# AKASH2907/pi-consistency-activity-detection

Measured on AMD Instinct MI355X. Metric: train clips/sec (bs=8, 16×224×224, I3D+caps+bv cons) at 1/2/4/8 GPU, higher is better.
Workload: dtype f32 (fp32 operands and fp32 accumulation everywhere; 33 of the 79 conv / input-gradient launches and the 3x3x3 / 1x1x1 weight gradients multiply on the bf16 matrix cores: every fp32 operand as the exact sum of 3 bf16 terms, 6 products on v_mfma_f32_32x32x16_bf16, hi / lo fp32 accumulators -- error v

## Files before the change

include/picons.h:

```cpp
#ifndef PICONS_H
#define PICONS_H
#include <stdint.h>
#ifdef __cplusplus
extern "C" {
#endif

typedef void* pc_stream;

#define PC_OK            0
#define PC_E_ARG        -1
#define PC_E_LAUNCH     -2
#define PC_E_NODEVICE   -3

#define PC_ACT_NONE 0
#define PC_ACT_RELU 1
#define PC_ACT_SIGMOID 2

#define PC_F_ACCUM   1
#define PC_F_BIAS    2
#define PC_F_CSCALE  4
#define PC_F_BNPART  8
#define PC_F_NFAST   16
#define PC_F_TOUT    32
#define PC_F_CI3     64
// ... 127 lines not shown
int64_t pc_act_bwd_ws_floats(int64_t rows, int C);
int pc_act_bwd(const float* dy, int lddy, const float* y, int ldy, int act, int C, int64_t rows,
               float* dz, int lddz, float* dbias, int accum, float* ws, pc_stream s);
int pc_ncdhw_to_ndhwc(const void* src, int src_is_f64, int N, int C, int64_t thw, int W, int Cpad,
                      int flipw, float* dst, pc_stream s);
int pc_ndhwc_to_ncdhw(const float* src, int ld, int N, int C, int64_t thw, float* dst, pc_stream s);
int pc_transpose_batched(const float* src, int batch, int R, int Cc, int64_t src_batch_stride,
                         int src_ld, float* dst, int64_t dst_batch_stride, int dst_ld, int accum,
                         pc_stream s);
typedef struct pc_transpose_job {
    uint64_t src, dst;
    int64_t  src_batch_stride, dst_batch_stride;
    int32_t  batch, R, C, src_ld, dst_ld, accum;
    int32_t  nslices, reserved;
    int64_t  slice_stride;
} pc_transpose_job;
int pc_transpose_multi(const pc_transpose_job* jobs, int njobs, pc_stream s);
int pc_col2im(const float* cols, int N, int Ho, int Wo, int KH, int KW, int C, float* dx, int lddx,
              int accum, pc_stream s);
int pc_seg_frame_counts(const float* logits, const float* gt, int64_t nframes, int64_t pix, int32_t* counts, pc_stream s);
int pc_map_accumulate(const int32_t* counts, int64_t nframes, int label, int ncls, int32_t* frame_hits, int32_t* video_hits,
                      int32_t* n_frames, int32_t* n_vids, pc_stream s);
int     pc_val_record_words(int B);
int64_t pc_val_metrics_ws_floats(int B, int64_t pix);
int     pc_val_metrics(const float* output, const float* loc_msk, const float* predicted_action, const int32_t* action, int B, int64_t pix,
                       int C, int32_t* record, float* ws, pc_stream s);
int pc_clip_from_u8(const uint8_t* video, int F, int H, int W, const int32_t* span8, int h0, int w0, int S,
                    const int32_t* rects, int R, float* data, float* aug, float* mask, pc_stream s);
int pc_clip_from_u8_masks(const uint8_t* video, int F, int H, int W, const int32_t* span8, int h0, int w0, int S,
                          const uint8_t* maskframes, const int32_t* valid8, float* data, float* aug, float* mask, float* mask_cls,
                          pc_stream s);
int pc_clip_from_u8_ndhwc4(const uint8_t* video, int F, int H, int W, const int32_t* span8, int h0, int w0, int S,
                           const int32_t* rects, int R, float* data, float* aug, float* mask, pc_stream s);
int pc_truth_frame_flags(const uint8_t* truth, int F, int H, int W, int h0, int w0, int S, int32_t* flags, pc_stream s);
int pc_eval_clips_from_u8(const uint8_t* video, const uint8_t* truth, int F, int H, int W, int h0, int w0, int S,
                          const int32_t* starts, int n, int f_skip, float* data, float* gt, pc_stream s);
int pc_video_vote(const float* pred, int n, int C, int label, int32_t* n_correct, pc_stream s);
int     pc_clips_from_u8(const uint8_t* video, int F, int H, int W, int h0, int w0, int S, const int32_t* starts, int n, int f_skip,
                         float* data, pc_stream s);
int64_t pc_detect_frames_ws_bytes(int n, int S);
int     pc_detect_frames(const float* logits, int F, int H, int W, int h0, int w0, int S, const int32_t* starts, int n, int f_skip,
                         int row0, uint8_t* mask, int32_t* rec, void* ws, pc_stream s);
int     pc_video_class(const float* scores, int n, int C, float* out, pc_stream s);
int     pc_clips_from_u8_views(const uint8_t* video, int F, int H, int W, int S, const int32_t* views, int V, int view_stride,
                               const int32_t* starts, int n, int f_skip, float* data, pc_stream s);
int64_t pc_detect_frames_views_ws_bytes(int n, int H, int W);
int     pc_detect_frames_views(const float* logits, int F, int H, int W, int S, const int32_t* views, int V, int view_stride,
                               const int32_t* starts, int n, int f_skip, int row0, uint8_t* mask, int32_t* rec, void* ws, pc_stream s);
#define PC_INST_HDR      4
#define PC_INST_WORDS    6
#define PC_INST_MAX_RUNS 2048
#define PC_INST_MAX_ROWS 2048
int     pc_frame_instances(const uint8_t* mask, int F, int H, int W, int f0, int nf, int conn, int min_area, int K, int32_t* inst,
                           uint8_t* imap, pc_stream s);
#define PC_PROB_ONE    65535
#define PC_SCORE_WORDS 3
int     pc_frame_probs(const float* logits, int F, int H, int W, int S, const int32_t* views, int V, int view_stride, const int32_t* starts,
                       int n, int f_skip, uint16_t* prob, pc_stream s);
int     pc_instance_scores(const uint8_t* imap, const uint16_t* prob, int F, int H, int W, int f0, int nf, int K, int32_t* out, pc_stream s);
#define PC_LINK_MAX_LAGS 4
int     pc_instance_overlaps(const uint8_t* imap, int F, int H, int W, int f0, int nf, int K, int L, int32_t* out, pc_stream s);
#define PC_RUN_WORDS 2
int64_t pc_mask_run_ws_bytes(int nf, int H);
int     pc_mask_run_index(const uint8_t* map, int F, int H, int W, int f0, int nf, int32_t* index, void* ws, pc_stream s);
int     pc_mask_runs(const uint8_t* map, int F, int H, int W, int f0, int nf, const int32_t* index, int64_t cap, uint32_t* runs, pc_stream s);
#define PC_CROSS_MAX_SLOTS 32
// ... 135 lines not shown
```

pi-consistency-activity-detection_amd/capi.py:

```python
import ctypes as C
import os

import numpy as np

_HERE = os.path.dirname(os.path.abspath(__file__))
DIAG = os.environ.get("PICONS_DIAG_LIB", "0") not in ("", "0")
DIAG_SWITCHES = ("PICONS_CONV_ABLATE", "PICONS_WGRAD_ABLATE", "PICONS_WINO_VARIANT")
LIB_PATH = os.path.join(_HERE, "libpicons_diag.so" if DIAG else "libpicons.so")
if os.environ.get("PICONS_LIB_NAME"):
    LIB_PATH = os.path.join(_HERE, os.path.basename(os.environ["PICONS_LIB_NAME"]))
_lib = None

i32, i64, f32, vp = C.c_int32, C.c_int64, C.c_float, C.c_void_p


class ConvDesc(C.Structure):
    _fields_ = [(n, i32) for n in ("N", "Ti", "Hi", "Wi", "Ci", "ldi", "Tq", "Hq", "Wq", "To", "Ho", "Wo", "Co", "ldo")] + \
               [(n, i32 * 3) for n in ("ostr", "ooff", "istr", "ntap", "ioff0", "istep", "wk0", "wkstep")] + \
               [(n, i32) for n in ("KT", "KH", "KW", "ldw", "act", "flags", "wgstride", "bgstride", "act_c0", "groups")]


class WgradDesc(C.Structure):
    _fields_ = [(n, i32) for n in ("N", "Tq", "Hq", "Wq", "Cd", "ldd", "Ts", "Hs", "Ws", "Cs", "lds")] + \
               [(n, i32 * 3) for n in ("istr", "ntap", "ioff0", "istep", "wk0")] + [(n, i32) for n in ("KT", "KH", "KW", "splitk", "nbatch", "dbstride", "sbstride", "gbstride", "Td", "Hd", "Wd")] + [("doff", i32 * 3), ("flags", i32), ("ws_slices", i32)]
# ... 74 lines not shown
    "pc_wino_weights": (i32, [vp, i64, i64, i64, i32, i32, i32, i32, vp, vp]),
    "pc_wino_weights_multi": (i32, [vp, i32, vp]),
    "pc_wino_conv": (i32, [C.POINTER(WinoDesc), vp, vp, vp, vp, vp, vp]),
    "pc_wino4_u_floats": (i64, [i32, i32, i32]),
    "pc_wino4_weights": (i32, [vp, i64, i64, i64, i32, i32, i32, i32, vp, vp]),
    "pc_wino_bnpart_rows": (i32, [C.POINTER(WinoDesc)]),
    "pc_wino_work": (i32, [C.POINTER(WinoDesc), C.POINTER(C.c_double)]),
    "pc_bn_finalize": (i32, [vp, i32, i32, i32, i64, vp, vp, f32, f32, vp, vp, vp, vp]),
    "pc_bn_finalize_ws": (i32, [vp, i32, i32, i32, i64, vp, vp, f32, f32, vp, vp, vp, vp, vp]),
    "pc_bn_finalize_ws_floats": (i64, [i32, i32, i32]),
    "pc_bn_finalize_apply_ok": (i32, [i32, i32]),
    "pc_bn_finalize_apply": (i32, [vp, i32, i32, i32, i64, vp, vp, f32, f32, vp, vp, vp, vp, i32, i64, vp, i32, i32, vp]),
    "pc_bn_apply": (i32, [vp, i32, vp, i32, i64, i32, vp, i32, i32, vp]),
    "pc_bn_eval_stat": (i32, [vp, vp, vp, vp, f32, i32, vp, vp]),
    "pc_bn_bwd_ws_floats": (i64, [i64, i32, i32]),
    "pc_bn_bwd": (i32, [vp, i32, vp, i32, vp, i32, i64, i32, i32, vp, i32, vp, vp, i32, vp, vp]),
    "pc_maxpool_fwd": (i32, [C.POINTER(PoolDesc), vp, vp, vp, vp]),
    "pc_maxpool_bwd": (i32, [C.POINTER(PoolDesc), vp, vp, vp, i32, vp]),
    "pc_channel_scale": (i32, [vp, i32, vp, i32, i64, i32, vp, i32, i32, vp]),
    "pc_act_bwd_ws_floats": (i64, [i64, i32]),
    "pc_act_bwd": (i32, [vp, i32, vp, i32, i32, i32, i64, vp, i32, vp, i32, vp, vp]),
    "pc_ncdhw_to_ndhwc": (i32, [vp, i32, i32, i32, i64, i32, i32, i32, vp, vp]),
    "pc_ndhwc_to_ncdhw": (i32, [vp, i32, i32, i32, i64, vp, vp]),
    "pc_transpose_batched": (i32, [vp, i32, i32, i32, i64, i32, vp, i64, i32, i32, vp]),
    "pc_col2im": (i32, [vp, i32, i32, i32, i32, i32, i32, vp, i32, i32, vp]),
    "pc_seg_frame_counts": (i32, [vp, vp, i64, i64, vp, vp]),
    "pc_map_accumulate": (i32, [vp, i64, i32, i32, vp, vp, vp, vp, vp]),
    "pc_val_record_words": (i32, [i32]),
    "pc_val_metrics_ws_floats": (i64, [i32, i64]),
    "pc_val_metrics": (i32, [vp, vp, vp, vp, i32, i64, i32, vp, vp, vp]),
    "pc_clip_from_u8": (i32, [vp, i32, i32, i32, C.POINTER(C.c_int32), i32, i32, i32, vp, i32, vp, vp, vp, vp]),
    "pc_clip_from_u8_ndhwc4": (i32, [vp, i32, i32, i32, C.POINTER(C.c_int32), i32, i32, i32, vp, i32, vp, vp, vp, vp]),
    "pc_clip_from_u8_masks": (i32, [vp, i32, i32, i32, C.POINTER(C.c_int32), i32, i32, i32, vp, C.POINTER(C.c_int32), vp, vp, vp, vp, vp]),
    "pc_truth_frame_flags": (i32, [vp, i32, i32, i32, i32, i32, i32, vp, vp]),
    "pc_eval_clips_from_u8": (i32, [vp, vp, i32, i32, i32, i32, i32, i32, C.POINTER(C.c_int32), i32, i32, vp, vp, vp]),
    "pc_video_vote": (i32, [vp, i32, i32, i32, vp, vp]),
    "pc_clips_from_u8": (i32, [vp, i32, i32, i32, i32, i32, i32, C.POINTER(C.c_int32), i32, i32, vp, vp]),
    "pc_detect_frames_ws_bytes": (i64, [i32, i32]),
    "pc_detect_frames": (i32, [vp, i32, i32, i32, i32, i32, i32, C.POINTER(C.c_int32), i32, i32, i32, vp, vp, vp, vp]),
    "pc_video_class": (i32, [vp, i32, i32, vp, vp]),
    "pc_clips_from_u8_views": (i32, [vp, i32, i32, i32, i32, C.POINTER(C.c_int32), i32, i32, C.POINTER(C.c_int32), i32, i32, vp, vp]),
    "pc_detect_frames_views_ws_bytes": (i64, [i32, i32, i32]),
    "pc_detect_frames_views": (i32, [vp, i32, i32, i32, i32, C.POINTER(C.c_int32), i32, i32, C.POINTER(C.c_int32), i32, i32, i32, vp, vp, vp, vp]),
    "pc_frame_instances": (i32, [vp, i32, i32, i32, i32, i32, i32, i32, i32, vp, vp, vp]),
    "pc_frame_probs": (i32, [vp, i32, i32, i32, i32, C.POINTER(C.c_int32), i32, i32, C.POINTER(C.c_int32), i32, i32, vp, vp]),
    "pc_instance_scores": (i32, [vp, vp, i32, i32, i32, i32, i32, i32, vp, vp]),
    "pc_instance_overlaps": (i32, [vp, i32, i32, i32, i32, i32, i32, i32, vp, vp]),
    "pc_mask_run_ws_bytes": (i64, [i32, i32]),
    "pc_mask_run_index": (i32, [vp, i32, i32, i32, i32, i32, vp, vp, vp]),
    "pc_mask_runs": (i32, [vp, i32, i32, i32, i32, i32, vp, i64, vp, vp]),
    "pc_map_crosstab_ws_bytes": (i64, [i32, i32, i32, i32, i32]),
    "pc_map_crosstab": (i32, [vp, vp, i32, i32, i32, i32, i32, i32, i32, vp, vp, vp]),
    "pc_resize_tables": (i64, [i32, i32, i32, i32, i32, vp, i64]),
    "pc_resize_u8": (i32, [vp, i32, i32, i32, i32, i32, i32, vp, i32, vp, vp]),
    "pc_fill": (i32, [vp, i64, f32, vp]),
    "pc_axpy": (i32, [vp, vp, i64, f32, vp]),
    "pc_em_ws_floats": (i64, [i32, i32, i32]),
    "pc_em_state_floats": (i64, [i32]),
    "pc_em_routing_fwd": (i32, [vp, vp, vp, vp, i32, i32, i32, vp, vp, vp]),
    "pc_em_routing_bwd": (i32, [vp, vp, vp, vp, vp, i32, i32, i32, vp, vp, vp, vp, vp, vp, vp]),
    "pc_class_mask_fwd": (i32, [vp, i32, i32, i32, vp, vp, i32, vp, vp, vp, vp]),
    "pc_class_mask_bwd": (i32, [vp, vp, vp, i32, i32, i32, vp, vp]),
    "pc_tapsum_fwd": (i32, [vp, i32, i32, i32, i32, vp, vp, vp]),
    "pc_tapsum_bwd": (i32, [vp, i32, i32, i32, i32, vp, vp]),
    "pc_loss_ws_floats": (i64, [C.POINTER(LossDesc)]),
    "pc_consistency_loss": (i32, [C.POINTER(LossDesc), vp, vp, vp, vp, vp, vp, vp, vp, vp, vp, vp]),
# ... 76 lines not shown
```

pi-consistency-activity-detection_amd/csrc/inputpipe.hip:

```cpp
#include "common.h"
#include <algorithm>
#include <cfloat>
#include <cmath>
#include <cstring>
#include <vector>

namespace {

struct ClipK {
    const uint8_t* video; int F, H, W;
    int span[8]; int h0, w0, S;
    const int32_t* rects; int R;
    const uint8_t* maskf; int valid[8]; float* mask_cls;
    float* data; float* aug; float* mask;
    int nhwc4;
};

__global__ __launch_bounds__(256) void clip_from_u8_kernel(const ClipK p) {
    const int S = p.S;
    const int64_t total = (int64_t)8 * S * S;
    for (int64_t idx = (int64_t)blockIdx.x * 256 + threadIdx.x; idx < total; idx += (int64_t)gridDim.x * 256) {
        const int w = (int)(idx % S), h = (int)((idx / S) % S), t = (int)(idx / ((int64_t)S * S));
        const int f = p.span[t], y = h + p.h0, x = w + p.w0;
        const uint8_t* px = p.video + (((size_t)f * p.H + y) * p.W + x) * 3;
// ... 33 lines not shown
                               const int32_t* rects, int R, float* data, float* aug, float* mask, pc_stream s) {
    return clip_launch(video, F, H, W, span8, h0, w0, S, rects, R, nullptr, nullptr, data, aug, mask, nullptr, s);
}

extern "C" int pc_clip_from_u8_masks(const uint8_t* video, int F, int H, int W, const int32_t* span8, int h0, int w0, int S,
                                     const uint8_t* maskframes, const int32_t* valid8, float* data, float* aug, float* mask, float* mask_cls,
                                     pc_stream s) {
    PC_CHECK_ARG(maskframes && valid8 && mask_cls, "pc_clip_from_u8_masks: null pointer");
    return clip_launch(video, F, H, W, span8, h0, w0, S, nullptr, 0, maskframes, valid8, data, aug, mask, mask_cls, s);
}

extern "C" int pc_clip_from_u8_ndhwc4(const uint8_t* video, int F, int H, int W, const int32_t* span8, int h0, int w0, int S,
                                      const int32_t* rects, int R, float* data, float* aug, float* mask, pc_stream s) {
    PC_CHECK_ARG(((uintptr_t)data % 16 == 0) && ((uintptr_t)aug % 16 == 0), "pc_clip_from_u8_ndhwc4: data / aug must be 16-byte aligned");
    return clip_launch(video, F, H, W, span8, h0, w0, S, rects, R, nullptr, nullptr, data, aug, mask, nullptr, s, 1);
}

static int clip_launch(const uint8_t* video, int F, int H, int W, const int32_t* span8, int h0, int w0, int S, const int32_t* rects, int R,
                       const uint8_t* maskf, const int32_t* valid8, float* data, float* aug, float* mask, float* mask_cls, pc_stream s, int nhwc4) {
    PC_CHECK_ARG(video && span8 && data && aug && mask && (rects || R == 0), "pc_clip_from_u8: null pointer");
    PC_CHECK_ARG(F >= 1 && S >= 1 && h0 >= 0 && w0 >= 0 && h0 + S <= H && w0 + S <= W && R >= 0, "pc_clip_from_u8: crop %d+%d x %d+%d outside %d x %d", h0, S, w0, S, H, W);
    ClipK k;
    k.video = video; k.F = F; k.H = H; k.W = W; k.h0 = h0; k.w0 = w0; k.S = S; k.rects = rects; k.R = R; k.data = data; k.aug = aug; k.mask = mask;
    k.maskf = maskf; k.mask_cls = mask_cls; k.nhwc4 = nhwc4;
    for (int t = 0; t < 8; ++t) k.valid[t] = valid8 ? valid8[t] : 0;
    for (int t = 0; t < 8; ++t) {
        PC_CHECK_ARG(span8[t] >= 0 && span8[t] < F, "pc_clip_from_u8: frame %d outside [0, %d)", span8[t], F);
        k.span[t] = span8[t];
    }
    const int64_t total = (int64_t)8 * S * S;
    int grid = (int)((total + 255) / 256); if (grid > 4096) grid = 4096;
    hipLaunchKernelGGL(clip_from_u8_kernel, dim3(grid), dim3(256), 0, (hipStream_t)s, k);
    PC_CHECK_LAUNCH("clip_from_u8");
    return PC_OK;
}

namespace {

enum { RK_NEAREST = 0, RK_LINEAR = 1, RK_AREA = 2, RK_AREA_FAST = 3, RK_COPY = 4 };
constexpr int RHDR = 8;

inline int cv_floor(double v) { int i = (int)v; return i - (i > v); }
inline int cv_ceil(double v) { int i = (int)v; return i + (i < v); }
inline int32_t fbits(float f) { int32_t b; memcpy(&b, &f, 4); return b; }
inline short sat_short(float v) { long r = lrintf(v); return (short)(r < -32768 ? -32768 : (r > 32767 ? 32767 : r)); }

void area_tab(int ssize, int dsize, double scale, std::vector<int32_t>& start, std::vector<int32_t>& si, std::vector<int32_t>& alpha) {
    for (int dx = 0; dx < dsize; ++dx) {
        start.push_back((int32_t)si.size());
        const double fsx1 = dx * scale, fsx2 = fsx1 + scale;
        const double cell = std::min(scale, ssize - fsx1);
        int sx1 = cv_ceil(fsx1), sx2 = cv_floor(fsx2);
        sx2 = std::min(sx2, ssize - 1);
        sx1 = std::min(sx1, sx2);
        if (sx1 - fsx1 > 1e-3) { si.push_back(sx1 - 1); alpha.push_back(fbits((float)((sx1 - fsx1) / cell))); }
        for (int sx = sx1; sx < sx2; ++sx) { si.push_back(sx); alpha.push_back(fbits(float(1.0 / cell))); }
        if (fsx2 - sx2 > 1e-3) { si.push_back(sx2); alpha.push_back(fbits((float)(std::min(std::min(fsx2 - sx2, 1.), cell) / cell))); }
    }
    start.push_back((int32_t)si.size());
}

struct ResizeK {
    const uint8_t* src; uint8_t* dst; const int32_t* tab;
    int n, H, W, C, Ho, Wo, binarize;
};

// ... 157 lines not shown
```

pi-consistency-activity-detection_amd/inputpipe.py:

```python
import numpy as np
import torch

from . import ops

DEPTH = 8
CROP = 224


class _PinnedRing:

    def __init__(self, depth=24):
        self.depth, self.buf, self.ev, self.nxt = depth, {}, {}, {}

    def _slot(self, shape, dtype):
        kind = (tuple(shape), str(dtype))
        i = self.nxt.get(kind, 0)
        self.nxt[kind] = (i + 1) % self.depth
        key = kind + (i,)
        if key not in self.buf:
            self.buf[key] = torch.empty(tuple(shape), dtype=torch.from_numpy(np.empty(0, dtype)).dtype).pin_memory()
            self.ev[key] = None
        if self.ev[key] is not None:
            self.ev[key].synchronize()
        return key, self.buf[key]

    def _send(self, key, b, device):
        d = b.to(device, non_blocking=True)
        ev = torch.cuda.Event()
        ev.record(torch.cuda.current_stream(d.device))
        self.ev[key] = ev
        return d

    def upload(self, frames, span, device):
        key, b = self._slot((len(span),) + tuple(frames.shape[1:]), frames.dtype)
        bn = b.numpy()
        for t, f in enumerate(span):
            bn[t] = frames[int(f)]
        return self._send(key, b, device)

    def upload_array(self, arr, device):
        key, b = self._slot(arr.shape, arr.dtype)
        b.numpy()[...] = arr
        return self._send(key, b, device)


_ring = _PinnedRing()


def pinned_upload(arr, device):
    return _ring.upload_array(np.ascontiguousarray(arr), device)


def frame_boxes(annotations, n_frames):
    if len(annotations) > 1:
        np.random.randint(0, len(annotations))
    per_frame = {}
    multi, label, labeled_vid = [], -1, -1
    for ann in annotations:
        multi.extend(ann[4])
        start_frame, end_frame, label, labeled_vid = ann[0], ann[1], ann[2], ann[5]
        for f in range(start_frame, min(n_frames, end_frame + 1)):
            per_frame.setdefault(f, []).append(ann[3][f - start_frame])
    return per_frame, label, list(set(multi)), labeled_vid


def frame_meta(annotations):
    if len(annotations) > 1:
        np.random.randint(0, len(annotations))
    multi, label, labeled_vid = [], -1, -1
    for ann in annotations:
        multi.extend(ann[4])
        label, labeled_vid = ann[2], ann[5]
    return label, list(set(multi)), labeled_vid


def boxes_of(annotations, n_frames, frame_ids):
    out = {}
    for f in frame_ids:
        f = int(f)
        for ann in annotations:
            if ann[0] <= f <= ann[1] and f < n_frames:
                out.setdefault(f, []).append(ann[3][f - ann[0]])
    return out
# ... 16 lines not shown
    if sel >= vlen:
        return None
    if start + (DEPTH * vskip) >= vlen:
        start = vlen - (DEPTH * vskip)
    return np.arange(DEPTH) * vskip + start


def _empty(device, size):
    z = torch.zeros(3, DEPTH, size, size, device=device)
    return {'data': z, 'loc_msk': torch.zeros(1, DEPTH, size, size, device=device), 'action': torch.Tensor([0]), 'aug_data': z, 'label_vid': 0}


def _resized_sample(video8, mask8, size):
    v = ops.resize_u8(video8, size, size, 1)
    m = ops.resize_u8(mask8, size, size, 1, binarize=True)
    data = (v.to(torch.float64) / 255.).to(torch.float32).permute(3, 0, 1, 2).contiguous()
    return data, torch.flip(data, [3]), m.to(torch.float32)


def get_item(frames, annotations, train=True, device="cuda", size=CROP, out=None, ndhwc4=False):
    if ndhwc4 and (out is None or size != CROP):
        raise ValueError("get_item: ndhwc4 is the staging layout of StepEngine.sample_stager (out=..., size 224)")

    def _into_out(e):
        if out is not None:
            for k, t in zip(("data", "aug_data", "loc_msk"), out):
                src = e[k]
                if ndhwc4 and k != "loc_msk":
                    t.zero_(); t[..., :3].copy_(src.permute(1, 2, 3, 0))
                else:
                    t.copy_(src.reshape(t.shape))
                e[k] = t
        return e
    if frames is None:
        return _into_out(_empty(device, size))
    vlen, clip_h, clip_w = int(frames.shape[0]), int(frames.shape[1]), int(frames.shape[2])
    label, annot_frames, labeled_vid = frame_meta(annotations)
    span = choose_window(annot_frames, vlen)
    if span is None:
        return _into_out(_empty(device, size))
    per_frame = boxes_of(annotations, vlen, span)
    if train:
        h0 = np.random.randint(0, clip_h - CROP); w0 = np.random.randint(0, clip_w - CROP)
    else:
        h0 = int((clip_h - CROP) / 2); w0 = int((clip_w - CROP) / 2)
    R = max([len(per_frame.get(int(f), [])) for f in span] + [1])
    rects = np.zeros((DEPTH, R, 4), np.int32)
    for t, f in enumerate(span):
        for r, (x, y, bw, bh) in enumerate(per_frame.get(int(f), [])):
            x0, x1, _ = slice(x, x + bw).indices(clip_w); y0, y1, _ = slice(y, y + bh).indices(clip_h)
            rects[t, r] = (x0, x1, y0, y1)
    if torch.is_tensor(frames):
        video, ids = frames.to(device), span
    else:
        video, ids = _ring.upload(frames, span, device), np.arange(DEPTH)
    rects_d = _ring.upload_array(rects, device)
    if size != CROP:
        crop8 = video.contiguous()[torch.as_tensor(np.asarray(ids), device=video.device).long(), h0:h0 + CROP, w0:w0 + CROP].contiguous()
        _d, _a, m224 = ops.clip_from_u8(video.contiguous(), ids, h0, w0, rects_d, CROP)
        data, aug, mask = _resized_sample(crop8, m224.to(torch.uint8), size)
        if out is not None:
            for src, t in zip((data, aug, mask), out):
                t.copy_(src.reshape(t.shape))
            data, aug, mask = out
    else:
        data, aug, mask = ops.clip_from_u8(video.contiguous(), ids, h0, w0, rects_d, CROP,
                                           out=None if out is None else (out[0], out[1], out[2].view(DEPTH, size, size)), ndhwc4=ndhwc4)
    return {'data': data, 'loc_msk': mask.view(1, DEPTH, size, size), 'action': torch.Tensor([label]), 'aug_data': aug, 'label_vid': labeled_vid}


def load_video_jhmdb(frames, part_mask, device="cuda"):
    f = (frames if torch.is_tensor(frames) else torch.from_numpy(np.ascontiguousarray(frames))).to(device).contiguous()
    pm = np.ascontiguousarray(np.transpose(np.asarray(part_mask), (2, 0, 1))) if not torch.is_tensor(part_mask) else part_mask.permute(2, 0, 1).contiguous()
    m = (pm if torch.is_tensor(pm) else torch.from_numpy(pm)).to(device).to(torch.uint8).contiguous()
    return ops.resize_u8(f, 256, 256, 3), ops.resize_u8(m, 256, 256, 0), np.arange(m.shape[0])


def get_item_jhmdb(frames, masks, label, annot_frames, train=True, device="cuda"):
    def empty():
        z = torch.zeros(3, DEPTH, CROP, CROP, device=device); m = torch.zeros(1, DEPTH, CROP, CROP, device=device)
        return {'data': z, 'loc_msk': m, 'action': torch.Tensor([0]), 'mask_cls': m.clone(), 'aug_data': z}
    if frames is None:
        return empty()
    vlen, clip_h, clip_w = int(frames.shape[0]), int(frames.shape[1]), int(frames.shape[2])
# ... 25 lines not shown
```

pi-consistency-activity-detection_amd/ops.py:

```python
import ctypes as C

import numpy as np
import torch

from . import capi, desc as D


def stream():
    return C.c_void_p(torch.cuda.current_stream().cuda_stream)


def ptr(t):
    if t is None:
        return None
    if not t.is_cuda:
        raise RuntimeError("picons ops need CUDA/HIP tensors (no CPU fallback)")
    return C.c_void_p(t.data_ptr())


def _fill_struct(st, d):
    for name, ctype in st._fields_:
        v = d[name]
        if isinstance(v, (list, tuple)):
            setattr(st, name, (C.c_int32 * 3)(*[int(x) for x in v]))
# ... 438 lines not shown
        record = torch.empty(max(val_record_words(B), 1), dtype=torch.int32, device=output.device)
    if ws is None:
        ws = torch.empty(max(val_metrics_ws_floats(B, pix), 4), dtype=torch.float32, device=output.device)
    capi.call("pc_val_metrics", ptr(output), ptr(loc_msk), ptr(predicted_action), ptr(action), B, pix, C_, ptr(record), ptr(ws), stream())
    return record


def decode_val_record(rec):
    r = np.ascontiguousarray(rec.cpu().numpy() if torch.is_tensor(rec) else rec, dtype=np.int32)
    B = int(r[9])
    out = {k: float(v) for k, v in zip(VAL_SCALARS, r[:8].view(np.float32))}
    out.update(n_correct=int(r[8]), B=B, counts=r[VAL_HEAD:VAL_HEAD + 3 * B].reshape(B, 3).copy())
    return out


def clip_from_u8(video, span, h0, w0, rects, S=224, out=None, ndhwc4=False):
    if video.dtype != torch.uint8 or video.dim() != 4 or video.shape[3] != 3 or not video.is_contiguous():
        raise ValueError("clip_from_u8: contiguous uint8 [F,H,W,3] frames")
    F, H, W, _ = video.shape
    R = 0 if rects is None else int(rects.shape[1])
    if rects is not None and (rects.dtype != torch.int32 or not rects.is_contiguous() or rects.shape[0] != 8 or rects.shape[2] != 4):
        raise ValueError("clip_from_u8: rects must be contiguous int32 [8,R,4]")
    nch = 4 if ndhwc4 else 3
    if out is None:
        data = torch.empty((8, S, S, 4) if ndhwc4 else (3, 8, S, S), device=video.device); aug = torch.empty_like(data); mask = torch.empty(8, S, S, device=video.device)
    else:
        data, aug, mask = out
        for t, n_ in ((data, nch * 8 * S * S), (aug, nch * 8 * S * S), (mask, 8 * S * S)):
            if t.dtype != torch.float32 or not t.is_contiguous() or t.numel() != n_ or t.device != video.device:
                raise ValueError("clip_from_u8: out tensors must be contiguous float32 device tensors of %d*8*S*S / %d*8*S*S / 8*S*S elements" % (nch, nch))
    sp = (C.c_int32 * 8)(*[int(v) for v in span])
    capi.call("pc_clip_from_u8_ndhwc4" if ndhwc4 else "pc_clip_from_u8", ptr(video), F, H, W, sp, int(h0), int(w0), S, ptr(rects) if R else None, R, ptr(data), ptr(aug), ptr(mask), stream())
    return data, aug, mask


def clip_from_u8_masks(video, span, h0, w0, maskframes, valid, S=224):
    if video.dtype != torch.uint8 or video.dim() != 4 or video.shape[3] != 3 or not video.is_contiguous():
        raise ValueError("clip_from_u8_masks: contiguous uint8 [F,H,W,3] frames")
    F, H, W, _ = video.shape
    if maskframes.dtype != torch.uint8 or tuple(maskframes.shape) != (F, H, W) or not maskframes.is_contiguous():
        raise ValueError("clip_from_u8_masks: maskframes must be contiguous uint8 [F,H,W]")
    data = torch.empty(3, 8, S, S, device=video.device); aug = torch.empty_like(data)
    mask = torch.empty(8, S, S, device=video.device); mask_cls = torch.empty_like(mask)
    sp = (C.c_int32 * 8)(*[int(v) for v in span]); va = (C.c_int32 * 8)(*[int(bool(v)) for v in valid])
    capi.call("pc_clip_from_u8_masks", ptr(video), F, H, W, sp, int(h0), int(w0), S, ptr(maskframes), va, ptr(data), ptr(aug), ptr(mask), ptr(mask_cls), stream())
    return data, aug, mask, mask_cls


def _u8_video(video, who, truth=None):
    if video.dtype != torch.uint8 or video.dim() != 4 or video.shape[3] != 3 or not video.is_contiguous():
        raise ValueError("%s: contiguous uint8 [F,H,W,3] frames" % who)
    if truth is not None and (truth.dtype != torch.uint8 or not truth.is_contiguous() or truth.numel() != video.numel() // 3
                              or tuple(truth.shape[:3]) != tuple(video.shape[:3])):
        raise ValueError("%s: truth must be contiguous uint8 [F,H,W] of the video's size" % who)
    return (int(v) for v in video.shape[:3])


def _starts_table(starts):
    n = len(starts)
    return (C.c_int32 * max(n, 1))(*[int(v) for v in starts]), n


def truth_frame_flags(truth, h0, w0, S, flags=None):
    if truth.dtype != torch.uint8 or truth.dim() != 3 or not truth.is_contiguous():
        raise ValueError("truth_frame_flags: contiguous uint8 [F,H,W] truth")
    F, H, W = (int(v) for v in truth.shape)
# ... 384 lines not shown
```

pi-consistency-activity-detection_amd/step.py:

```python
import ctypes as C
import os
from collections import OrderedDict
from types import SimpleNamespace

import numpy as np
import torch

from . import capi, ops, spec, switches as sw, synthetic
from .plan import Plan


def default_args(**kw):
    a = dict(bv=False, gv=False, n_frames=3, predict_maps=False, lower_thresh=None, upper_thresh=None,
             bv_wt=0.5, gv_wt=0.5, wt_loc=1.0, wt_cls=1.0, wt_cons=1.0, thresh_epoch=11, lr=1e-3, epochs=1)
    a.update(kw)
    return SimpleNamespace(**a)


def exp_rampup(rampup_length):
    def f(epoch):
        if epoch < rampup_length:
            e = float(np.clip(epoch, 0.0, rampup_length))
            ph = 1.0 - e / rampup_length
            return float(np.exp(-5.0 * ph * ph))
        return 1.0
    return f


class StepEngine:

    SHORT_PLANS = 2

    def __init__(self, args, bs=8, hw=224, num_classes=24, device="cuda:0", jhmdb=False, state=None, seed=47, lanes=None, exp=None):
        if not torch.cuda.is_available():
            raise RuntimeError("StepEngine needs a GPU: the hot path is HIP-only (no CPU fallback)")
        capi.lib()
        self.args = args
        self.exp = dict(exp or {})
        self.dev = torch.device(device)
        torch.cuda.set_device(self.dev)
        self.bs = bs
# ... 528 lines not shown
    def _commit_small(self, slot):
        eng, p, n = self.eng, self.eng.active, self.m[slot]
        per = spec.FRAMES * eng.hw * eng.hw
        eng.aview(p.in_seg, n * per).copy_(self.dev[slot]["loc_msk"][:n].reshape(-1))
        ds = self.dev_small[slot]
        eng.aview(p.in_cls, 2 * n).copy_(torch.cat([ds[:n], ds[:n]]))
        eng.aview(p.in_labeled, 2 * n, torch.int32).copy_(torch.cat([ds[n:2 * n], ds[n:2 * n]]).to(torch.int32))
        o, c8 = 2 * n, n * spec.TRUNK_OUT_CH
        eng.aview(p.in_drop832, 2 * c8).copy_(ds[o:o + 2 * c8])
        eng.aview(p.in_drop128, 2 * n * 128).copy_(ds[o + 2 * c8:o + 2 * c8 + 2 * n * 128])
        eng.labels_host, eng.action_host = self.host[slot]

    def release(self, slot):
        self.consumed[slot].record(torch.cuda.current_stream(self.eng.dev))


class SampleStager(HostDictStager):

    def __init__(self, eng):
        eng._activate(eng.bs)
        super().__init__(eng, dtype=torch.float32, host=False)
        n, hw, T = eng.bs, eng.hw, spec.FRAMES
        p = eng.plan
        lane = int(sw.get("PICONS_STAGE_LANE", "1"))
        self.stage_stream = eng.side[lane - 1] if 1 <= lane <= len(eng.side) else self.copy_stream
        self.x = [torch.empty(2 * n, T, hw, hw, 4, dtype=torch.float32, device=eng.dev) for _ in range(2)]
        for d in self.dev:
            d.pop("data"); d.pop("aug_data")
        self.o_cls, self.o_lab, self.o_d832 = 0, 2 * n, 4 * n
        self.o_d128 = self.o_d832 + 2 * n * spec.TRUNK_OUT_CH
        self.nsmall = self.o_d128 + 2 * n * 128
        self.pin_small = [torch.empty(self.nsmall, dtype=torch.float32).pin_memory() for _ in range(2)]
        self.dev_small = [torch.empty(self.nsmall, dtype=torch.float32, device=eng.dev) for _ in range(2)]
        if not hasattr(eng, "_patched"):
            conv_ops = tuple(("fwd", idx) for idx in p.op_to_ndhwc)
            per = T * hw * hw
            eng._patched = dict(img=eng.readers_of(p.img.ref, 2 * n * per * 4, skip=conv_ops), seg=eng.readers_of(p.in_seg, n * per),
                                cls=eng.readers_of(p.in_cls, 2 * n), lab=eng.readers_of(p.in_labeled, 2 * n),
                                d832=eng.readers_of(p.in_drop832, 2 * n * spec.TRUNK_OUT_CH), d128=eng.readers_of(p.in_drop128, 2 * n * 128))
            if not eng._patched["img"][1] or not eng._patched["seg"][1]:
                raise RuntimeError("no op reads the clip tensor / the mask: the plan changed under SampleStager")
            kinds = {(name, int(eng.ops[name][idx]["kind"])) for name, idx, _q, _o in eng._patched["img"][1]}
            if ("fwd", capi.OP_CONV) not in kinds or (p.training and ("bwd", capi.OP_WGRAD) not in kinds):
                raise RuntimeError("SampleStager: the stem's conv / weight gradient are not among the clip's readers (%s)" % sorted(kinds))

    def _pack_small(self, slot, act, lab_flag, drops):
        n = self.eng.bs
        T_ = lambda a: a if torch.is_tensor(a) else torch.from_numpy(np.asarray(a))
        ps = self.pin_small[slot]
        ps[self.o_cls:self.o_cls + n] = act; ps[self.o_cls + n:self.o_cls + 2 * n] = act
        li = ps.view(torch.int32)
        li[self.o_lab:self.o_lab + n] = lab_flag.to(torch.int32); li[self.o_lab + n:self.o_lab + 2 * n] = lab_flag.to(torch.int32)
        o = self.o_d832
        for d, c in zip((drops[0], drops[2], drops[1], drops[3]), (spec.TRUNK_OUT_CH, spec.TRUNK_OUT_CH, 128, 128)):
            ps[o:o + n * c] = T_(d).reshape(-1).float()
            o += n * c
        self.host[slot] = (lab_flag.to(torch.int32), act.clone())

    def prepare(self, slot, make_sample, nl, perm, drops):
        eng, n = self.eng, self.eng.bs
        perm = np.asarray(perm)
        if perm.shape != (n,) or not 1 <= nl < n:
            raise ValueError("SampleStager stages full minibatches only: %d clips (%d labeled) on an engine built for %d" % (perm.size, nl, n))
        eng._check_perm_drops(n, perm, drops)
        where = np.empty(n, np.int64)
        where[perm] = np.arange(n)
        x, m = self.x[slot], self.dev[slot]["loc_msk"]
        st_ = self.stage_stream
        with torch.cuda.stream(st_):
            if self.used[slot]:
                st_.wait_event(self.consumed[slot])
            samples = [make_sample(i, (x[where[i]], x[n + where[i]], m[where[i]])) for i in range(n)]
            act = torch.tensor([float(torch.as_tensor(smp["action"]).reshape(-1)[0]) for smp in samples])[perm]
            if eng.jhmdb:
                lab_flag = torch.cat([torch.ones(nl), torch.zeros(n - nl)])[perm]
            else:
                lab_flag = torch.tensor([float(smp["label_vid"]) for smp in samples])[perm]
            self._pack_small(slot, act, lab_flag, drops)
            self.dev_small[slot].copy_(self.pin_small[slot], non_blocking=True)
            self.ready[slot].record(st_)
        self.used[slot] = True

    def commit(self, slot):
        eng, p = self.eng, self.eng.plan
        torch.cuda.current_stream(eng.dev).wait_event(self.ready[slot])
        eng._activate(eng.bs)
        for idx in p.op_to_ndhwc:
            eng.ops["fwd"][idx]["i"][1] = 0
        ds = self.dev_small[slot].data_ptr()
        where = dict(img=self.x[slot].data_ptr(), seg=self.dev[slot]["loc_msk"].data_ptr(), cls=ds + 4 * self.o_cls, lab=ds + 4 * self.o_lab,
                     d832=ds + 4 * self.o_d832, d128=ds + 4 * self.o_d128)
        for key, (_base, readers) in eng._patched.items():
            for name, idx, q, offb in readers:
                eng.ops[name][idx]["p"][q] = where[key] + offb
        eng.labels_host, eng.action_host = self.host[slot]
```

Baseline: 454.0.

## Batch clip staging into one pinned slab upload and single decode kernel

Instead of each sample uploading its own uint8 frames and launching its own crop/convert kernel, samples are packed into one pinned host slab (frames, rectangles and small per-batch tensors), copied with a single async H2D transfer, and decoded by one batched kernel that writes data, flipped aug and masks for all clips. This removes per-sample launches and small transfers in the staging path. It adds a host synchronize on the slot's ready event before reuse, and the slab can be reallocated with a full device sync if it grows.

Result: no change. 453.0 (-0.2%).

```diff
diff --git a/include/picons.h b/include/picons.h
--- a/include/picons.h
+++ b/include/picons.h
@@ -183,6 +183,12 @@
                           pc_stream s);
 int pc_clip_from_u8_ndhwc4(const uint8_t* video, int F, int H, int W, const int32_t* span8, int h0, int w0, int S,
                            const int32_t* rects, int R, float* data, float* aug, float* mask, pc_stream s);
+#define PC_CLIP_BATCH_MAX 32
+typedef struct pc_clip_sample {
+    int32_t H, W, frames_off, h0, w0, rects_off, R, j, empty, reserved;
+} pc_clip_sample;
+int pc_clips_from_u8_batch(const uint8_t* slab, int64_t slab_bytes, const pc_clip_sample* samples, int n, float* clips, float* mask,
+                           int cap, int S, pc_stream s);
 int pc_truth_frame_flags(const uint8_t* truth, int F, int H, int W, int h0, int w0, int S, int32_t* flags, pc_stream s);
 int pc_eval_clips_from_u8(const uint8_t* video, const uint8_t* truth, int F, int H, int W, int h0, int w0, int S,
                           const int32_t* starts, int n, int f_skip, float* data, float* gt, pc_stream s);
diff --git a/pi-consistency-activity-detection_amd/capi.py b/pi-consistency-activity-detection_amd/capi.py
--- a/pi-consistency-activity-detection_amd/capi.py
+++ b/pi-consistency-activity-detection_amd/capi.py
@@ -130,6 +130,7 @@
     "pc_clip_from_u8": (i32, [vp, i32, i32, i32, C.POINTER(C.c_int32), i32, i32, i32, vp, i32, vp, vp, vp, vp]),
     "pc_clip_from_u8_ndhwc4": (i32, [vp, i32, i32, i32, C.POINTER(C.c_int32), i32, i32, i32, vp, i32, vp, vp, vp, vp]),
     "pc_clip_from_u8_masks": (i32, [vp, i32, i32, i32, C.POINTER(C.c_int32), i32, i32, i32, vp, C.POINTER(C.c_int32), vp, vp, vp, vp, vp]),
+    "pc_clips_from_u8_batch": (i32, [vp, i64, vp, i32, vp, vp, i32, i32, vp]),
     "pc_truth_frame_flags": (i32, [vp, i32, i32, i32, i32, i32, i32, vp, vp]),
     "pc_eval_clips_from_u8": (i32, [vp, vp, i32, i32, i32, i32, i32, i32, C.POINTER(C.c_int32), i32, i32, vp, vp, vp]),
     "pc_video_vote": (i32, [vp, i32, i32, i32, vp, vp]),
diff --git a/pi-consistency-activity-detection_amd/csrc/inputpipe.hip b/pi-consistency-activity-detection_amd/csrc/inputpipe.hip
--- a/pi-consistency-activity-detection_amd/csrc/inputpipe.hip
+++ b/pi-consistency-activity-detection_amd/csrc/inputpipe.hip
@@ -89,6 +89,124 @@
     int grid = (int)((total + 255) / 256); if (grid > 4096) grid = 4096;
     hipLaunchKernelGGL(clip_from_u8_kernel, dim3(grid), dim3(256), 0, (hipStream_t)s, k);
     PC_CHECK_LAUNCH("clip_from_u8");
+    return PC_OK;
+}
+
+namespace {
+
+constexpr int CB_ROWS = 8;
+constexpr int CB_RECTS = 64;
+
+struct ClipBatchK {
+    const uint8_t* slab; float4* clips; float* mask;
+    int cap, S;
+    pc_clip_sample smp[PC_CLIP_BATCH_MAX];
+};
+
+struct __attribute__((packed)) px4_bytes { uint8_t b[12]; };
+
+__device__ __forceinline__ float in_rect(const int4 r, int x, int y) {
+    return (x >= r.x && x < r.y && y >= r.z && y < r.w) ? 1.f : 0.f;
+}
+
+__global__ __launch_bounds__(256) void clips_from_u8_batch_kernel(const ClipBatchK p) {
+    __shared__ float lut[256];
+    __shared__ int4 rc[CB_RECTS];
+    const pc_clip_sample& d = p.smp[blockIdx.z];
+    const int tid = threadIdx.y * 64 + threadIdx.x;
+    const int t = blockIdx.y, S = p.S;
+    const bool empty = d.empty != 0;
+    const int R = empty ? 0 : d.R, Rl = R < CB_RECTS ? R : CB_RECTS;
+    const int4* rects = (const int4*)(p.slab + d.rects_off) + (size_t)t * R;
+    lut[tid] = (float)((double)tid / 255.0);
+    if (tid < Rl) rc[tid] = rects[tid];
+    __syncthreads();
+    const size_t per = (size_t)S * S;
+    const size_t at = ((size_t)d.j * 8 + t) * per;
+    float4* data = p.clips + at;
+    float4* aug = p.clips + (size_t)p.cap * 8 * per + at;
+    float* mask = p.mask + at;
+    const uint8_t* fr = p.slab + d.frames_off + ((size_t)t * d.H + d.h0) * d.W * 3 + (size_t)d.w0 * 3;
+    const size_t pitch = (size_t)d.W * 3;
+    const int Q = S >> 2;
+    const bool vec_mask = (S & 3) == 0;
+    const int h1 = min(S, ((int)blockIdx.x + 1) * CB_ROWS);
+    for (int h = blockIdx.x * CB_ROWS + threadIdx.y; h < h1; h += 4) {
+        const int y = h + d.h0;
+        const uint8_t* src = fr + (size_t)h * pitch;
+        float4* drow = data + (size_t)h * S;
+        float4* arow = aug + (size_t)h * S + (S - 1);
+        float* mrow = mask + (size_t)h * S;
+        for (int w = threadIdx.x * 4; w < Q * 4; w += 256) {
+            px4_bytes px = {};
+            if (!empty) px = *(const px4_bytes*)(src + w * 3);
+            const int x = w + d.w0;
+            float4 m = make_float4(0.f, 0.f, 0.f, 0.f);
+            for (int q = 0; q < Rl; ++q) {
+                const int4 r = rc[q];
+                m.x = fmaxf(m.x, in_rect(r, x, y)); m.y = fmaxf(m.y, in_rect(r, x + 1, y));
+                m.z = fmaxf(m.z, in_rect(r, x + 2, y)); m.w = fmaxf(m.w, in_rect(r, x + 3, y));
+            }
+            for (int q = Rl; q < R; ++q) {
+                const int4 r = rects[q];
+                m.x = fmaxf(m.x, in_rect(r, x, y)); m.y = fmaxf(m.y, in_rect(r, x + 1, y));
+                m.z = fmaxf(m.z, in_rect(r, x + 2, y)); m.w = fmaxf(m.w, in_rect(r, x + 3, y));
+            }
+#pragma unroll
+            for (int k = 0; k < 4; ++k) {
+                const float4 v = make_float4(lut[px.b[3 * k]], lut[px.b[3 * k + 1]], lut[px.b[3 * k + 2]], 0.f);
+                drow[w + k] = v;
+                arow[-(w + k)] = v;
+            }
+            if (vec_mask) *(float4*)(mrow + w) = m;
+            else { mrow[w] = m.x; mrow[w + 1] = m.y; mrow[w + 2] = m.z; mrow[w + 3] = m.w; }
+        }
+        for (int w = Q * 4 + threadIdx.x; w < S; w += 64) {
+            const uint8_t* px = src + w * 3;
+            const float4 v = empty ? make_float4(0.f, 0.f, 0.f, 0.f) : make_float4(lut[px[0]], lut[px[1]], lut[px[2]], 0.f);
+            drow[w] = v;
+            arow[-w] = v;
+            const int x = w + d.w0;
+            float m = 0.f;
+            for (int q = 0; q < Rl; ++q) m = fmaxf(m, in_rect(rc[q], x, y));
+            for (int q = Rl; q < R; ++q) m = fmaxf(m, in_rect(rects[q], x, y));
+            mrow[w] = m;
+        }
+    }
+}
+
+}
+
+extern "C" int pc_clips_from_u8_batch(const uint8_t* slab, int64_t slab_bytes, const pc_clip_sample* samples, int n, float* clips, float* mask,
+                                      int cap, int S, pc_stream s) {
+    const char* who = "pc_clips_from_u8_batch";
+    PC_CHECK_ARG(slab && samples && clips && mask, "%s: null pointer", who);
+    PC_CHECK_ARG((uintptr_t)slab % 16 == 0 && (uintptr_t)clips % 16 == 0 && (uintptr_t)mask % 16 == 0, "%s: slab / clips / mask must be 16-byte aligned", who);
+    PC_CHECK_ARG(n >= 1 && n <= PC_CLIP_BATCH_MAX, "%s: %d samples outside 1..%d", who, n, PC_CLIP_BATCH_MAX);
+    PC_CHECK_ARG(cap >= 1 && S >= 1 && S <= 32768 && slab_bytes >= 0, "%s: cap = %d, S = %d, slab of %lld bytes", who, cap, S, (long long)slab_bytes);
+    ClipBatchK k;
+    memset(&k, 0, sizeof(k));
+    for (int i = 0; i < n; ++i) {
+        const pc_clip_sample& d = samples[i];
+        PC_CHECK_ARG(d.j >= 0 && d.j < cap, "%s: sample %d at position %d outside the %d of the minibatch", who, i, d.j, cap);
+        for (int q = 0; q < i; ++q)
+            PC_CHECK_ARG(samples[q].j != d.j, "%s: samples %d and %d at the same position %d", who, q, i, d.j);
+        PC_CHECK_ARG(d.R >= 0, "%s: sample %d with R = %d rectangles", who, i, d.R);
+        k.smp[i].j = d.j;
+        k.smp[i].empty = d.empty != 0;
+        if (d.empty) continue;
+        k.smp[i] = d;
+        PC_CHECK_ARG(d.H >= 1 && d.W >= 1 && d.h0 >= 0 && d.w0 >= 0 && (int64_t)d.h0 + S <= d.H && (int64_t)d.w0 + S <= d.W,
+                     "%s: sample %d: crop %d+%d x %d+%d outside %d x %d", who, i, d.h0, S, d.w0, S, d.H, d.W);
+        PC_CHECK_ARG(d.H <= 32768 && d.W <= 32768 && d.frames_off >= 0 && (int64_t)d.frames_off + (int64_t)8 * d.H * d.W * 3 <= slab_bytes,
+                     "%s: sample %d: 8 frames of %d x %d at byte %d outside the slab's %lld bytes", who, i, d.H, d.W, d.frames_off, (long long)slab_bytes);
+        PC_CHECK_ARG(d.R == 0 || (d.rects_off >= 0 && d.rects_off % 16 == 0 && (int64_t)d.rects_off + (int64_t)8 * d.R * 16 <= slab_bytes),
+                     "%s: sample %d: %d rectangles per frame at byte %d outside the slab's %lld bytes (or not on 16 bytes)", who, i, d.R, d.rects_off,
+                     (long long)slab_bytes);
+    }
+    k.slab = slab; k.clips = (float4*)clips; k.mask = mask; k.cap = cap; k.S = S;
+    hipLaunchKernelGGL(clips_from_u8_batch_kernel, dim3((unsigned)cdiv(S, CB_ROWS), 8, (unsigned)n), dim3(64, 4), 0, (hipStream_t)s, k);
+    PC_CHECK_LAUNCH(who);
     return PC_OK;
 }
 
diff --git a/pi-consistency-activity-detection_amd/inputpipe.py b/pi-consistency-activity-detection_amd/inputpipe.py
--- a/pi-consistency-activity-detection_amd/inputpipe.py
+++ b/pi-consistency-activity-detection_amd/inputpipe.py
@@ -49,6 +49,89 @@
 
 def pinned_upload(arr, device):
     return _ring.upload_array(np.ascontiguousarray(arr), device)
+
+
+def _align16(v):
+    return (int(v) + 15) & ~15
+
+
+class ClipBatch:
+
+    RECT_ROOM = 1024
+
+    def __init__(self, device, head_bytes, n, frames_hw=(240, 320)):
+        self.device = torch.device(device)
+        self.head = _align16(head_bytes)
+        self.pin = self.dev = self.x = self.m = None
+        self.used, self.cap, self.desc, self.rects = self.head, 0, [], []
+        self.grown = 0
+        self._alloc(self.head + n * (_align16(DEPTH * frames_hw[0] * frames_hw[1] * 3) + self.RECT_ROOM))
+
+    def _alloc(self, nbytes):
+        old = self.pin
+        torch.cuda.synchronize(self.device)
+        self.pin = torch.empty(int(nbytes), dtype=torch.uint8).pin_memory()
+        self.dev = torch.empty(int(nbytes), dtype=torch.uint8, device=self.device)
+        self.np = self.pin.numpy()
+        if old is not None:
+            self.np[:self.used] = old.numpy()[:self.used]
+            self.grown += 1
+
+    def _room(self, nbytes, samples_left=0, sample_bytes=0):
+        if nbytes > self.pin.numel():
+            self._alloc(nbytes + samples_left * sample_bytes + max(self.cap * self.RECT_ROOM, sum(_align16(r.nbytes) for r in self.rects if r is not None)))
+
+    def begin(self, x, m, cap):
+        self.x, self.m, self.cap = x, m, int(cap)
+        self.used, self.desc, self.rects = self.head, [], []
+
+    def position(self, out):
+        per = DEPTH * CROP * CROP
+        d, a, m = out
+        if self.x is None or any(t.dtype != torch.float32 or not t.is_contiguous() for t in out) or d.numel() != 4 * per or a.numel() != 4 * per or m.numel() != per:
+            return None
+        off = d.data_ptr() - self.x.data_ptr()
+        j = off // (16 * per)
+        if off < 0 or off % (16 * per) or j >= self.cap:
+            return None
+        if a.data_ptr() != self.x.data_ptr() + (self.cap + j) * 16 * per or m.data_ptr() != self.m.data_ptr() + j * 4 * per:
+            return None
+        if any(row[7] == j for row in self.desc):
+            raise ValueError("get_item: position %d of the minibatch is written twice" % j)
+        return int(j)
+
+    def add(self, j, frames, span, h0, w0, rects):
+        H, W = int(frames.shape[1]), int(frames.shape[2])
+        nb = DEPTH * H * W * 3
+        off = self.used
+        self._room(off + _align16(nb), self.cap - len(self.desc) - 1, _align16(nb))
+        dst = self.np[off:off + nb].reshape(DEPTH, H, W, 3)
+        for t, f in enumerate(span):
+            dst[t] = frames[int(f)]
+        self.used = off + _align16(nb)
+        self.desc.append([H, W, off, int(h0), int(w0), 0, int(rects.shape[1]), j, 0, 0])
+        self.rects.append(np.ascontiguousarray(rects, np.int32))
+
+    def add_empty(self, j):
+        self.desc.append([0, 0, 0, 0, 0, 0, 0, j, 1, 0])
+        self.rects.append(None)
+
+    def close(self):
+        self._room(self.used + sum(_align16(r.nbytes) for r in self.rects if r is not None))
+        for row, r in zip(self.desc, self.rects):
+            if r is not None and r.size:
+                row[5] = self.used
+                self.np[self.used:self.used + r.nbytes] = r.reshape(-1).view(np.uint8)
+                self.used += _align16(r.nbytes)
+
+    def flush(self):
+        self.dev[:self.used].copy_(self.pin[:self.used], non_blocking=True)
+        for i in range(0, len(self.desc), ops.CLIP_BATCH_MAX):
+            ops.clips_from_u8_batch(self.dev, np.asarray(self.desc[i:i + ops.CLIP_BATCH_MAX], np.int32), self.x, self.m, self.cap, CROP, slab_bytes=self.used)
+        self.x = self.m = None
+
+
+_open_batch = None
 
 
 def frame_boxes(annotations, n_frames):
@@ -131,13 +214,20 @@
                     t.copy_(src.reshape(t.shape))
                 e[k] = t
         return e
+    slot_j = _open_batch.position(out) if (ndhwc4 and _open_batch is not None) else None
+
+    def _zero_sample():
+        if slot_j is None:
+            return _into_out(_empty(device, size))
+        _open_batch.add_empty(slot_j)
+        return {'data': out[0], 'loc_msk': out[2], 'action': torch.Tensor([0]), 'aug_data': out[1], 'label_vid': 0}
     if frames is None:
-        return _into_out(_empty(device, size))
+        return _zero_sample()
     vlen, clip_h, clip_w = int(frames.shape[0]), int(frames.shape[1]), int(frames.shape[2])
     label, annot_frames, labeled_vid = frame_meta(annotations)
     span = choose_window(annot_frames, vlen)
     if span is None:
-        return _into_out(_empty(device, size))
+        return _zero_sample()
     per_frame = boxes_of(annotations, vlen, span)
     if train:
         h0 = np.random.randint(0, clip_h - CROP); w0 = np.random.randint(0, clip_w - CROP)
@@ -149,6 +239,9 @@
         for r, (x, y, bw, bh) in enumerate(per_frame.get(int(f), [])):
             x0, x1, _ = slice(x, x + bw).indices(clip_w); y0, y1, _ = slice(y, y + bh).indices(clip_h)
             rects[t, r] = (x0, x1, y0, y1)
+    if slot_j is not None and isinstance(frames, np.ndarray) and frames.dtype == np.uint8 and frames.ndim == 4 and frames.shape[3] == 3:
+        _open_batch.add(slot_j, frames, span, h0, w0, rects)
+        return {'data': out[0], 'loc_msk': out[2], 'action': torch.Tensor([label]), 'aug_data': out[1], 'label_vid': labeled_vid}
     if torch.is_tensor(frames):
         video, ids = frames.to(device), span
     else:
diff --git a/pi-consistency-activity-detection_amd/ops.py b/pi-consistency-activity-detection_amd/ops.py
--- a/pi-consistency-activity-detection_amd/ops.py
+++ b/pi-consistency-activity-detection_amd/ops.py
@@ -494,6 +494,24 @@
     sp = (C.c_int32 * 8)(*[int(v) for v in span])
     capi.call("pc_clip_from_u8_ndhwc4" if ndhwc4 else "pc_clip_from_u8", ptr(video), F, H, W, sp, int(h0), int(w0), S, ptr(rects) if R else None, R, ptr(data), ptr(aug), ptr(mask), stream())
     return data, aug, mask
+
+
+CLIP_BATCH_MAX = 32
+CLIP_SAMPLE_FIELDS = ("H", "W", "frames_off", "h0", "w0", "rects_off", "R", "j", "empty", "reserved")
+
+
+def clips_from_u8_batch(slab, samples, clips, mask, cap, S=224, slab_bytes=None):
+    if slab.dtype != torch.uint8 or not slab.is_contiguous():
+        raise ValueError("clips_from_u8_batch: the slab must be a contiguous uint8 device tensor")
+    smp = np.ascontiguousarray(samples, dtype=np.int32)
+    if smp.ndim != 2 or smp.shape[1] != len(CLIP_SAMPLE_FIELDS):
+        raise ValueError("clips_from_u8_batch: samples must be int32 [n, %d] (%s)" % (len(CLIP_SAMPLE_FIELDS), ", ".join(CLIP_SAMPLE_FIELDS)))
+    cap, S = int(cap), int(S)
+    for t, n_ in ((clips, 2 * cap * 8 * S * S * 4), (mask, cap * 8 * S * S)):
+        if t.dtype != torch.float32 or not t.is_contiguous() or t.numel() < n_ or t.device != slab.device:
+            raise ValueError("clips_from_u8_batch: clips / mask must be contiguous float32 device tensors of at least 2*cap*8*S*S*4 / cap*8*S*S elements")
+    capi.call("pc_clips_from_u8_batch", ptr(slab), int(slab.numel() if slab_bytes is None else slab_bytes), smp.ctypes.data_as(C.c_void_p),
+              int(smp.shape[0]), ptr(clips), ptr(mask), cap, S, stream())
 
 
 def clip_from_u8_masks(video, span, h0, w0, maskframes, valid, S=224):
diff --git a/pi-consistency-activity-detection_amd/step.py b/pi-consistency-activity-detection_amd/step.py
--- a/pi-consistency-activity-detection_amd/step.py
+++ b/pi-consistency-activity-detection_amd/step.py
@@ -6,7 +6,7 @@
 import numpy as np
 import torch
 
-from . import capi, ops, spec, switches as sw, synthetic
+from . import capi, inputpipe, ops, spec, switches as sw, synthetic
 from .plan import Plan
 
 
@@ -601,6 +601,8 @@
         self.nsmall = self.o_d128 + 2 * n * 128
         self.pin_small = [torch.empty(self.nsmall, dtype=torch.float32).pin_memory() for _ in range(2)]
         self.dev_small = [torch.empty(self.nsmall, dtype=torch.float32, device=eng.dev) for _ in range(2)]
+        self._own_small = (list(self.pin_small), list(self.dev_small))
+        self.batch = [inputpipe.ClipBatch(eng.dev, 4 * self.nsmall, n) for _ in range(2)]
         if not hasattr(eng, "_patched"):
             conv_ops = tuple(("fwd", idx) for idx in p.op_to_ndhwc)
             per = T * hw * hw
@@ -636,17 +638,34 @@
         where[perm] = np.arange(n)
         x, m = self.x[slot], self.dev[slot]["loc_msk"]
         st_ = self.stage_stream
+        b = self.batch[slot] if sw.get("PICONS_STAGE_BATCH", "1") not in ("", "0") else None
+        if b is not None and self.used[slot]:
+            self.ready[slot].synchronize()
         with torch.cuda.stream(st_):
             if self.used[slot]:
                 st_.wait_event(self.consumed[slot])
-            samples = [make_sample(i, (x[where[i]], x[n + where[i]], m[where[i]])) for i in range(n)]
+            if b is not None:
+                b.begin(x, m, n)
+                inputpipe._open_batch = b
+            try:
+                samples = [make_sample(i, (x[where[i]], x[n + where[i]], m[where[i]])) for i in range(n)]
+            finally:
+                inputpipe._open_batch = None
             act = torch.tensor([float(torch.as_tensor(smp["action"]).reshape(-1)[0]) for smp in samples])[perm]
             if eng.jhmdb:
                 lab_flag = torch.cat([torch.ones(nl), torch.zeros(n - nl)])[perm]
             else:
                 lab_flag = torch.tensor([float(smp["label_vid"]) for smp in samples])[perm]
-            self._pack_small(slot, act, lab_flag, drops)
-            self.dev_small[slot].copy_(self.pin_small[slot], non_blocking=True)
+            if b is not None:
+                b.close()
+                self.pin_small[slot] = b.pin[:4 * self.nsmall].view(torch.float32)
+                self.dev_small[slot] = b.dev[:4 * self.nsmall].view(torch.float32)
+                self._pack_small(slot, act, lab_flag, drops)
+                b.flush()
+            else:
+                self.pin_small[slot], self.dev_small[slot] = self._own_small[0][slot], self._own_small[1][slot]
+                self._pack_small(slot, act, lab_flag, drops)
+                self.dev_small[slot].copy_(self.pin_small[slot], non_blocking=True)
             self.ready[slot].record(st_)
         self.used[slot] = True
 
```
